# nathanaelbosch/ODEFilters.jl

Hardware: AMD Instinct MI355X
Metric: ensemble ODE-filter steps/sec (whole node) (higher is better)
Workload: dtype f64

## Files before the change

odefilters.jl_amd/csrc/ek_kernels.h:

```cpp
#pragma once
#include <hip/hip_runtime.h>
#include "dispatch.h"
#include "smooth_rows.h"
#include "smooth_lane.h"
#include "dense_lane.h"
#include "sample_lane.h"
#include "rows_kernels.h"
#include "dense_rows.h"
#include "sample_rows.h"
#include "launch.h"
#include "wave_map.h"

namespace odef {

constexpr int kWave = 64;
inline unsigned lane_grid(long N) { return (unsigned)((N + kWave - 1) / kWave); }

__device__ __attribute__((always_inline)) inline void stagger_start(const FilterParams& P) {
  if (P.stagger > 0) {
    const int n = (int)(blockIdx.x % 16u) * P.stagger;
    for (int k = 0; k < n; ++k) __builtin_amdgcn_s_sleep(1);
  }
}
template <class RHS, int q, bool EK1, bool EVERY, bool LAG = false>
__global__ __launch_bounds__(kWave) void ek_filter_fixed_kernel(const FilterParams P) {
  const long i0 = wave_first_trajectory(blockIdx.x, gridDim.x, P.wave_map);
  stagger_start(P);
  if (i0 + threadIdx.x < P.N) filter_fixed_lane<RHS, q, EK1, EVERY, LAG>(P, i0, threadIdx.x);
}
template <class RHS, int q, bool EK1>
__global__ __launch_bounds__(kWave) void ek_filter_adaptive_kernel(const FilterParams P) {
  const long i0 = (long)blockIdx.x * kWave;
  if (i0 + threadIdx.x < P.N) filter_adaptive_lane<RHS, q, EK1>(P, i0, threadIdx.x);
}
template <class RHS, int q, bool EVERY, bool LAG>
__global__ __launch_bounds__(kWave) void ek_filter_fixed_mv_kernel(const FilterParams P) {
  const long i0 = wave_first_trajectory(blockIdx.x, gridDim.x, P.wave_map);
  stagger_start(P);
  if (i0 + threadIdx.x < P.N) filter_fixed_lane<RHS, q, false, EVERY, LAG, true>(P, i0, threadIdx.x);
}
template <class RHS, int q>
__global__ __launch_bounds__(kWave) void ek_filter_adaptive_mv_kernel(const FilterParams P) {
  const long i0 = (long)blockIdx.x * kWave;
  if (i0 + threadIdx.x < P.N) filter_adaptive_lane<RHS, q, false, true>(P, i0, threadIdx.x);
}
template <class RHS, int q, bool LAG>
__global__ __launch_bounds__(kWave) void ek_filter_fixed_ieks_kernel(const FilterParams P) {
  const long i0 = wave_first_trajectory(blockIdx.x, gridDim.x, P.wave_map);
  stagger_start(P);
  if (i0 + threadIdx.x < P.N) filter_fixed_lane<RHS, q, true, true, LAG, false, true>(P, i0, threadIdx.x);
}

template <int D>
struct SmoothTeam {
  static constexpr int lanes = (D <= 16) ? 16 : 32;
  static unsigned grid(long items) { return (unsigned)((items + kWave / lanes - 1) / (kWave / lanes)); }
};
template <int d, int q, bool MV>
__device__ __attribute__((always_inline)) inline void smooth_team_entry(const SmoothParams& P) {
  constexpr int D = d * (q + 1), TEAM = SmoothTeam<D>::lanes, TPB = kWave / TEAM;
  using W = RowsWs<d, q + 1>;
  __shared__ double lds[TPB * W::size];
  const int team = threadIdx.x / TEAM, tid = threadIdx.x % TEAM;
  const long i = (long)blockIdx.x * TPB + team;
  RowState<D> st;
  if (i < P.N) smooth_rows_lane<d, q, TEAM, MV>(P, i, tid, lds + team * W::size, &st);
}
template <int d, int q>
__global__ __launch_bounds__(kWave) __attribute__((amdgpu_num_vgpr(128))) void rts_smooth_kernel(const SmoothParams P) {
  smooth_team_entry<d, q, false>(P);
}
template <int d, int q>
__global__ __launch_bounds__(kWave) __attribute__((amdgpu_num_vgpr(128))) void rts_smooth_mv_kernel(const SmoothParams P) {
  smooth_team_entry<d, q, true>(P);
}
constexpr int kSmoothLaneMaxD = 12;
constexpr long kSmoothLaneMinN = 6144;
inline long smooth_lane_min_n() { return env_long("ODEF_SMOOTH_LANE_MIN_N", kSmoothLaneMinN); }
constexpr long kFilterLagMaxN = kFilterRowsMaxN;
inline long filter_lag_max_n() { return env_long("ODEF_FILTER_LAG_MAX_N", kFilterLagMaxN); }
static_assert(kWaveMapLanes == kWave, "wave_map.h counts trajectories in wavefronts of the lane kernels");
constexpr long kWaveMapDefault = 1;
inline int wave_map_mode() { return (int)env_long("ODEF_WAVE_MAP", kWaveMapDefault); }
template <int d, int q, bool ADAPT>
__global__ __launch_bounds__(kWave) void rts_smooth_lane_kernel(const SmoothParams P) {
  constexpr int D = d * (q + 1), TRI = D * (D + 1) / 2;
  __shared__ double lds[TRI * kWave];
  const long i0 = (long)blockIdx.x * kWave;
  const LaneMem xl{lds + threadIdx.x, kWave};
  const bool valid = i0 + threadIdx.x < P.N;
  long n_hi = P.n_save;
  if constexpr (ADAPT) n_hi = wave_uniform_max(valid ? (long)P.nsaved[i0 + threadIdx.x] : 0, valid);
  if (valid) smooth_lane_v2<d, q, ADAPT>(P, i0, threadIdx.x, xl, n_hi);
}

template <int d, int q>
__global__ __launch_bounds__(kWave) void dense_output_kernel(const DenseParams P) {
  constexpr int D = d * (q + 1), TRI = D * (D + 1) / 2;
  __shared__ double lds[TRI * kWave];
  const long i = (long)blockIdx.x * kWave + threadIdx.x;
  const LaneMem xl{lds + threadIdx.x, kWave};
  if (i < P.N) dense_lane<d, q>(P, i, (long)blockIdx.y, xl);
}
template <int d, int q>
__global__ __launch_bounds__(kWave) void dense_output_mv_kernel(const DenseParams P) {
  constexpr int D = d * (q + 1), TRI = D * (D + 1) / 2;
  __shared__ double lds[TRI * kWave];
  const long i = (long)blockIdx.x * kWave + threadIdx.x;
  const LaneMem xl{lds + threadIdx.x, kWave};
  if (i < P.N) dense_lane<d, q, true>(P, i, (long)blockIdx.y, xl);
}
template <int d, int q, bool MV>
__device__ __attribute__((always_inline)) inline void dense_team_entry(const DenseParams& P) {
  constexpr int D = d * (q + 1), TEAM = SmoothTeam<D>::lanes, TPB = kWave / TEAM;
  using W = RowsWs<d, q + 1>;
  __shared__ double lds[TPB * W::size];
  const int team = threadIdx.x / TEAM, tid = threadIdx.x % TEAM;
  const long it = (long)blockIdx.x * TPB + team;
  RowState<D> st;
  if (it < P.N * P.n_q) dense_rows_lane<d, q, TEAM, MV>(P, it % P.N, it / P.N, tid, lds + team * W::size, &st);
}
template <int d, int q>
__global__ __launch_bounds__(kWave) __attribute__((amdgpu_num_vgpr(128))) void dense_rows_kernel(const DenseParams P) {
  dense_team_entry<d, q, false>(P);
}
template <int d, int q>
__global__ __launch_bounds__(kWave) __attribute__((amdgpu_num_vgpr(128))) void dense_rows_mv_kernel(const DenseParams P) {
  dense_team_entry<d, q, true>(P);
}

template <int d, int q>
__global__ __launch_bounds__(kWave) void sample_kernel(const SampleParams P) {
  constexpr int D = d * (q + 1), TRI = D * (D + 1) / 2;
  __shared__ double lds[TRI * kWave];
  const long i = (long)blockIdx.x * kWave + threadIdx.x;
  const LaneMem xl{lds + threadIdx.x, kWave};
  const bool valid = i < P.N;
  const long n_hi = (P.adaptive && !P.tq) ? wave_uniform_max(valid ? (long)P.nsaved[i] : 0, valid) : P.n_save;
  if (valid) sample_lane<d, q>(P, i, (long)blockIdx.y, xl, n_hi);
}
template <int d, int q>
__global__ __launch_bounds__(kWave) void sample_mv_kernel(const SampleParams P) {
  constexpr int D = d * (q + 1), TRI = D * (D + 1) / 2;
  __shared__ double lds[TRI * kWave];
  const long i = (long)blockIdx.x * kWave + threadIdx.x;
  const LaneMem xl{lds + threadIdx.x, kWave};
  const bool valid = i < P.N;
  const long n_hi = (P.adaptive && !P.tq) ? wave_uniform_max(valid ? (long)P.nsaved[i] : 0, valid) : P.n_save;
  if (valid) sample_lane<d, q, true>(P, i, (long)blockIdx.y, xl, n_hi);
}
template <int d, int q, bool MV>
__device__ __attribute__((always_inline)) inline void sample_team_entry(const SampleParams& P) {
  constexpr int D = d * (q + 1), TEAM = SmoothTeam<D>::lanes, TPB = kWave / TEAM;
  using W = RowsWs<d, q + 1>;
  __shared__ double lds[TPB * W::size];
  const int team = threadIdx.x / TEAM, tid = threadIdx.x % TEAM;
  const long it = (long)blockIdx.x * TPB + team;
  RowState<D> st;
  if (it < P.N * P.n_samples) sample_rows_lane<d, q, TEAM, MV>(P, it % P.N, it / P.N, tid, lds + team * W::size, &st);
}
template <int d, int q>
__global__ __launch_bounds__(kWave) __attribute__((amdgpu_num_vgpr(128))) void sample_rows_kernel(const SampleParams P) {
  sample_team_entry<d, q, false>(P);
}
template <int d, int q>
__global__ __launch_bounds__(kWave) __attribute__((amdgpu_num_vgpr(128))) void sample_rows_mv_kernel(const SampleParams P) {
  sample_team_entry<d, q, true>(P);
}

template <bool WITH_MV = true>
struct LaunchDenseT {
  const DenseParams& P;
  hipStream_t s;
  int rc = 0;
  template <int d, int q>
  void operator()() {
    if (P.mv) {
      if constexpr (WITH_MV) launch<d, q, true>();
      else rc = -2;
      return;
    }
    launch<d, q, false>();
  }
  template <int d, int q, bool MV>
  void launch() {
    constexpr int D = d * (q + 1);
    if constexpr (D <= kSmoothLaneMaxD) {
      const dim3 grid(lane_grid(P.N), (unsigned)P.n_q);
      if constexpr (MV) hipLaunchKernelGGL((dense_output_mv_kernel<d, q>), grid, dim3(kWave), 0, s, P);
      else hipLaunchKernelGGL((dense_output_kernel<d, q>), grid, dim3(kWave), 0, s, P);
    } else if constexpr (D <= 32) {
      const dim3 grid(SmoothTeam<D>::grid(P.N * P.n_q));
      if constexpr (MV) hipLaunchKernelGGL((dense_rows_mv_kernel<d, q>), grid, dim3(kWave), 0, s, P);
      else hipLaunchKernelGGL((dense_rows_kernel<d, q>), grid, dim3(kWave), 0, s, P);
    } else {
      rc = MV ? -2 : -3;
    }
  }
};
template <bool WITH_MV = true>
struct LaunchSampleT {
  const SampleParams& P;
  hipStream_t s;
  int rc = 0;
  template <int d, int q>
  void operator()() {
    if (P.mv) {
      if constexpr (WITH_MV) launch<d, q, true>();
      else rc = -2;
      return;
    }
    launch<d, q, false>();
  }
  template <int d, int q, bool MV>
  void launch() {
    constexpr int D = d * (q + 1);
    if constexpr (D <= kSmoothLaneMaxD) {
      const dim3 grid(lane_grid(P.N), (unsigned)P.n_samples);
      if constexpr (MV) hipLaunchKernelGGL((sample_mv_kernel<d, q>), grid, dim3(kWave), 0, s, P);
      else hipLaunchKernelGGL((sample_kernel<d, q>), grid, dim3(kWave), 0, s, P);
    } else if constexpr (D <= 32) {
      const dim3 grid(SmoothTeam<D>::grid(P.N * P.n_samples));
      if constexpr (MV) hipLaunchKernelGGL((sample_rows_mv_kernel<d, q>), grid, dim3(kWave), 0, s, P);
      else hipLaunchKernelGGL((sample_rows_kernel<d, q>), grid, dim3(kWave), 0, s, P);
    } else {
      rc = MV ? -2 : -3;
    }
  }
};
template <bool WITH_MV = true>
struct LaunchSmoothT {
  const SmoothParams& P;
  hipStream_t s;
  int rc = 0;
  template <int d, int q>
  void operator()() {
    if (P.mv) {
      if constexpr (WITH_MV && d * (q + 1) <= 32) launch<d, q, true>();
      else rc = -2;
      return;
    }
    launch<d, q, false>();
  }
  template <int d, int q, bool MV>
  void launch() {
    constexpr int D = d * (q + 1);
    if constexpr (!MV && D <= kRowsMaxD) {
      if (P.N < smooth_rows_max_n()) {
        const dim3 grid(rows_grid(P.N));
        note_kernel("odef::rts_smooth_bcast_kernel<%d, %d, %s>", d, q, tf(P.adaptive));
        if (P.adaptive) hipLaunchKernelGGL((rts_smooth_bcast_kernel<d, q, true>), grid, dim3(kRowsBlock), 0, s, P);
        else hipLaunchKernelGGL((rts_smooth_bcast_kernel<d, q, false>), grid, dim3(kRowsBlock), 0, s, P);
        return;
      }
    }
    if constexpr (!MV && D <= kSmoothLaneMaxD) {
      if (P.N >= smooth_lane_min_n()) {
        const dim3 grid(lane_grid(P.N));
        note_kernel("odef::rts_smooth_lane_kernel<%d, %d, %s>", d, q, tf(P.adaptive));
        if (P.adaptive) hipLaunchKernelGGL((rts_smooth_lane_kernel<d, q, true>), grid, dim3(kWave), 0, s, P);
        else hipLaunchKernelGGL((rts_smooth_lane_kernel<d, q, false>), grid, dim3(kWave), 0, s, P);
        return;
      }
    }
    const dim3 grid(SmoothTeam<D>::grid(P.N));
    note_kernel(MV ? "odef::rts_smooth_mv_kernel<%d, %d>" : "odef::rts_smooth_kernel<%d, %d>", d, q);
    if constexpr (MV) hipLaunchKernelGGL((rts_smooth_mv_kernel<d, q>), grid, dim3(kWave), 0, s, P);
    else hipLaunchKernelGGL((rts_smooth_kernel<d, q>), grid, dim3(kWave), 0, s, P);
  }
};
template <bool WITH_MV = true, bool WITH_IEKS = true>
struct LaunchFilterT {
  const FilterParams& P;
  int adaptive;
  hipStream_t s;
  int rc = 0;
  enum Mode { kScalar, kMv, kIeks };
  template <class RHS, int q, bool EK1>
  void operator()() {
    const bool mv = P.fixed_diffusion >= 3;
    if (P.lin) {
      if constexpr (WITH_IEKS && EK1) {
        if (!adaptive && P.everystep && !mv) return launch<RHS, q, EK1, kIeks>();
      }
      rc = -2;
    } else if (mv) {
      if constexpr (WITH_MV && !EK1) launch<RHS, q, EK1, kMv>();
      else rc = -2;
    } else {
      launch<RHS, q, EK1, kScalar>();
    }
  }
  template <class RHS, int q, bool EK1, Mode M>
  void launch() {
    if constexpr (RHS::d * (q + 1) <= kRowsMaxD && M != kMv) {
      if (P.N < filter_rows_max_n()) {
        const dim3 grid(rows_grid(P.N));
        if constexpr (M == kIeks) {
          note_kernel("odef::ek_filter_rows_ieks_kernel<odef::%s, %d>", RHS::name, q);
          hipLaunchKernelGGL((ek_filter_rows_ieks_kernel<RHS, q>), grid, dim3(kRowsBlock), 0, s, P);
        } else if (adaptive) {
          note_kernel("odef::ek_filter_rows_adaptive_kernel<odef::%s, %d, %s>", RHS::name, q, tf(EK1));
          hipLaunchKernelGGL((ek_filter_rows_adaptive_kernel<RHS, q, EK1>), grid, dim3(kRowsBlock), 0, s, P);
        } else {
          note_kernel("odef::ek_filter_rows_kernel<odef::%s, %d, %s, %s>", RHS::name, q, tf(EK1), tf(P.everystep));
          if (P.everystep) hipLaunchKernelGGL((ek_filter_rows_kernel<RHS, q, EK1, true>), grid, dim3(kRowsBlock), 0, s, P);
          else hipLaunchKernelGGL((ek_filter_rows_kernel<RHS, q, EK1, false>), grid, dim3(kRowsBlock), 0, s, P);
        }
        return;
      }
    }
    const dim3 grid(lane_grid(P.N));
    if constexpr (M != kIeks) {
      if (adaptive) {
        if constexpr (M == kMv) {
          note_kernel("odef::ek_filter_adaptive_mv_kernel<odef::%s, %d>", RHS::name, q);
          hipLaunchKernelGGL((ek_filter_adaptive_mv_kernel<RHS, q>), grid, dim3(kWave), 0, s, P);
        } else {
          note_kernel("odef::ek_filter_adaptive_kernel<odef::%s, %d, %s>", RHS::name, q, tf(EK1));
          hipLaunchKernelGGL((ek_filter_adaptive_kernel<RHS, q, EK1>), grid, dim3(kWave), 0, s, P);
        }
        return;
      }
    }
    const bool lag = P.everystep && P.N < filter_lag_max_n();
    FilterParams Pw = P;
    Pw.wave_map = wave_map_mode();
    if constexpr (M == kIeks) {
      note_kernel("odef::ek_filter_fixed_ieks_kernel<odef::%s, %d, %s>", RHS::name, q, tf(lag));
      if (lag) hipLaunchKernelGGL((ek_filter_fixed_ieks_kernel<RHS, q, true>), grid, dim3(kWave), 0, s, Pw);
      else hipLaunchKernelGGL((ek_filter_fixed_ieks_kernel<RHS, q, false>), grid, dim3(kWave), 0, s, Pw);
    } else if constexpr (M == kMv) {
      note_kernel("odef::ek_filter_fixed_mv_kernel<odef::%s, %d, %s, %s>", RHS::name, q, tf(P.everystep), tf(lag));
      if (lag) hipLaunchKernelGGL((ek_filter_fixed_mv_kernel<RHS, q, true, true>), grid, dim3(kWave), 0, s, Pw);
      else if (P.everystep) hipLaunchKernelGGL((ek_filter_fixed_mv_kernel<RHS, q, true, false>), grid, dim3(kWave), 0, s, Pw);
      else hipLaunchKernelGGL((ek_filter_fixed_mv_kernel<RHS, q, false, false>), grid, dim3(kWave), 0, s, Pw);
    } else {
      note_kernel("odef::ek_filter_fixed_kernel<odef::%s, %d, %s, %s, %s>", RHS::name, q, tf(EK1), tf(P.everystep), tf(lag));
      if (lag) hipLaunchKernelGGL((ek_filter_fixed_kernel<RHS, q, EK1, true, true>), grid, dim3(kWave), 0, s, Pw);
      else if (P.everystep) hipLaunchKernelGGL((ek_filter_fixed_kernel<RHS, q, EK1, true>), grid, dim3(kWave), 0, s, Pw);
      else hipLaunchKernelGGL((ek_filter_fixed_kernel<RHS, q, EK1, false>), grid, dim3(kWave), 0, s, Pw);
    }
  }
};

template <class RHS, int ONLYQ = 0, bool ONLYEK1 = false, bool WITH_MV = true, bool WITH_IEKS = true>
int lane_filter(int q, int ek1, const FilterParams& P, hipStream_t s, int adaptive, double*, size_t, long*) {
  LaunchFilterT<WITH_MV, WITH_IEKS> f{P, adaptive, s};
  const int rc = dispatch_order<RHS, ONLYQ, ONLYEK1>(q, ek1, f);
  return rc ? rc : f.rc;
}
template <int d, int ONLYQ = 0, bool WITH_MV = true>
int lane_smooth(int q, const SmoothParams& P, double*, hipStream_t s) {
  LaunchSmoothT<WITH_MV> f{P, s};
  const int rc = dispatch_smooth_order<d, ONLYQ>(q, f);
  return rc ? rc : f.rc;
}
template <int d, int ONLYQ = 0, bool WITH_MV = true>
int lane_dense(int q, const DenseParams& P, double*, hipStream_t s) {
  LaunchDenseT<WITH_MV> f{P, s};
  const int rc = dispatch_smooth_order<d, ONLYQ>(q, f);
  return rc ? rc : f.rc;
}
template <int d, int ONLYQ = 0, bool WITH_MV = true>
int lane_sample(int q, const SampleParams& P, double*, hipStream_t s) {
  LaunchSampleT<WITH_MV> f{P, s};
  const int rc = dispatch_smooth_order<d, ONLYQ>(q, f);
  return rc ? rc : f.rc;
}
extern template int lane_smooth<2>(int, const SmoothParams&, double*, hipStream_t);
extern template int lane_dense<2>(int, const DenseParams&, double*, hipStream_t);
extern template int lane_sample<2>(int, const SampleParams&, double*, hipStream_t);
extern template int lane_smooth<3>(int, const SmoothParams&, double*, hipStream_t);
extern template int lane_dense<3>(int, const DenseParams&, double*, hipStream_t);
extern template int lane_sample<3>(int, const SampleParams&, double*, hipStream_t);

}
```

odefilters.jl_amd/csrc/smooth_lane.h:

```cpp
#pragma once
#include "ek_lane.h"

namespace odef {

struct LaneMem {
  double* base;
  int stride;
  __device__ inline double get(int k) const { return base[k * stride]; }
  __device__ inline void set(int k, double v) const { base[k * stride] = v; }
};

template <int D>
__device__ inline void two_sided_inverse(double (&S)[D * (D + 1) / 2], const double (&L)[D * (D + 1) / 2], const double (&dinv)[D]) {
  static_for<0, D>([&](auto kc) {
    constexpr int k = decltype(kc)::value;
    const double inv = dinv[k];
    const double tkk = S[tri(k, k)] * inv * inv;
    S[tri(k, k)] = tkk;
    const double htkk = -0.5 * tkk;
#pragma unroll
    for (int j = 0; j < k; ++j) S[tri(k, j)] *= inv;
    double b[D];
#pragma unroll
    for (int i = k + 1; i < D; ++i) {
      const double lik = L[tri(i, k)];
      b[i] = __builtin_fma(lik, htkk, S[tri(i, k)] * inv);
#pragma unroll
      for (int j = 0; j < k; ++j) S[tri(i, j)] = __builtin_fma(-lik, S[tri(k, j)], S[tri(i, j)]);
    }
#pragma unroll
    for (int i = k + 1; i < D; ++i) {
      const double lik = L[tri(i, k)];
#pragma unroll
      for (int j = k + 1; j <= i; ++j)
        S[tri(i, j)] = __builtin_fma(-L[tri(j, k)], b[i], __builtin_fma(-lik, b[j], S[tri(i, j)]));
      S[tri(i, k)] = __builtin_fma(lik, htkk, b[i]);
    }
    ODEF_SCHED_FENCE();
  });
  static_for<0, D>([&](auto kc) {
    constexpr int k = D - 1 - decltype(kc)::value;
    const double inv = dinv[k];
    double t[D];
#pragma unroll
    for (int j = 0; j < D; ++j) {
      double s = S[symidx(k, j)];
#pragma unroll
      for (int i = k + 1; i < D; ++i) s -= L[tri(i, k)] * S[symidx(i, j)];
      t[j] = s;
    }
    double tk = t[k];
#pragma unroll
    for (int i = k + 1; i < D; ++i) tk -= L[tri(i, k)] * t[i];
#pragma unroll
    for (int j = 0; j < D; ++j)
      if (j != k) S[symidx(k, j)] = t[j] * inv;
    S[tri(k, k)] = tk * inv * inv;
    ODEF_SCHED_FENCE();
  });
}

template <int d, int NB>
__device__ inline void congruence_At_inplace(const PriorConsts& pc, double (&X)[d * NB * (d * NB + 1) / 2]) {
  constexpr int D = d * NB;
#pragma unroll
  for (int J = NB - 1; J >= 1; --J) {
    double Wd[d][d];
#pragma unroll
    for (int a = 0; a < d; ++a)
#pragma unroll
      for (int b = 0; b < d; ++b) {
        double t = X[symidx(J * d + a, J * d + b)];
#pragma unroll
        for (int j = 0; j < J; ++j) t += pc.At[j][J] * X[symidx(j * d + a, J * d + b)];
        Wd[a][b] = t;
      }
#pragma unroll
    for (int a = 0; a < d; ++a)
#pragma unroll
      for (int c = 0; c < D; ++c) {
        if (c / d == J) continue;
        double t = X[symidx(J * d + a, c)];
#pragma unroll
        for (int j = 0; j < J; ++j) t += pc.At[j][J] * X[symidx(j * d + a, c)];
        X[symidx(J * d + a, c)] = t;
      }
#pragma unroll
    for (int a = 0; a < d; ++a)
#pragma unroll
      for (int b = 0; b <= a; ++b) {
        double t = Wd[a][b];
#pragma unroll
        for (int j = 0; j < J; ++j) t += pc.At[j][J] * X[symidx(J * d + a, j * d + b)];
        X[tri(J * d + a, J * d + b)] = t;
      }
  }
}

template <int d, int NB, class CovSink, class Sig = double>
__device__ inline void rts_step_core(const PriorConsts& pc, const double (&pij)[NB], const double (&mt)[d * NB],
                                     double (&B)[d * NB * (d * NB + 1) / 2], double (&Cs)[d * NB * (d * NB + 1) / 2],
                                     const double (&msn)[d * NB], Sig sigma2, const LaneMem& xl,
                                     double (&ms_out)[d * NB], CovSink& sink) {
  constexpr int D = d * NB, TRI = D * (D + 1) / 2;
  double dl[D];
#pragma unroll
  for (int J = 0; J < NB; ++J)
#pragma unroll
    for (int a = 0; a < d; ++a) {
      double t = mt[J * d + a];
#pragma unroll
      for (int j = J + 1; j < NB; ++j) t += pc.At[J][j] * mt[j * d + a];
      dl[J * d + a] = msn[J * d + a] - t;
    }
  ODEF_SCHED_FENCE();
  predict_cov_inplace<d, NB>(pc, B, sigma2);
  ODEF_SCHED_FENCE();
#pragma unroll
  for (int k = 0; k < TRI; ++k) Cs[k] -= B[k];
  int fixes = 0;
  double dinv[D];
  chol_packed<D>(B, fixes, dinv);
  ODEF_SCHED_FENCE();
#pragma unroll
  for (int k = 0; k < D; ++k) {
    double t = dl[k];
#pragma unroll
    for (int c = 0; c < k; ++c) t -= B[tri(k, c)] * dl[c];
    dl[k] = t * dinv[k];
  }
#pragma unroll
  for (int k = D - 1; k >= 0; --k) {
    double t = dl[k];
#pragma unroll
    for (int c = k + 1; c < D; ++c) t -= B[tri(c, k)] * dl[c];
    dl[k] = t * dinv[k];
  }
  double wv[D];
#pragma unroll
  for (int K = 0; K < NB; ++K)
#pragma unroll
    for (int b = 0; b < d; ++b) {
      double t = dl[K * d + b];
#pragma unroll
      for (int j = 0; j < K; ++j) t += pc.At[j][K] * dl[j * d + b];
      wv[K * d + b] = t;
    }
  ODEF_SCHED_FENCE();
  two_sided_inverse<D>(Cs, B, dinv);
  ODEF_SCHED_FENCE();
  congruence_At_inplace<d, NB>(pc, Cs);
  ODEF_SCHED_FENCE();
  static_for<0, D>([&](auto ac) {
    constexpr int a = decltype(ac)::value;
    double xa[D], u[D];
#pragma unroll
    for (int c = 0; c < D; ++c) xa[c] = xl.get(symidx(a, c));
    double mnew = mt[a];
#pragma unroll
    for (int c = 0; c < D; ++c) mnew += xa[c] * wv[c];
    ms_out[a] = mnew * pij[a / d];
#pragma unroll
    for (int c = 0; c < D; ++c) {
      double t = 0.0;
#pragma unroll
      for (int k = 0; k < D; ++k) t += xa[k] * Cs[symidx(k, c)];
      u[c] = t;
    }
#pragma unroll
    for (int b = 0; b <= a; ++b) {
      double t = xa[b];
#pragma unroll
      for (int k = 0; k < D; ++k) t += u[k] * xl.get(symidx(k, b));
      sink(tri(a, b), t * (pij[a / d] * pij[b / d]));
    }
    ODEF_SCHED_FENCE();
  });
}

__device__ inline long wave_uniform_max(long v, bool valid) {
#ifdef ODEF_HOST_EMUL
  (void)valid;
  return v;
#else
  int x = valid ? (int)v : 0;
  for (int m = 32; m >= 1; m >>= 1) {
    const int y = __shfl_xor(x, m, 64);
    x = x > y ? x : y;
  }
  return (long)__builtin_amdgcn_readfirstlane(x);
#endif
}

#ifdef ODEF_HOST_EMUL
inline double* agpr_file() {
  static thread_local double f[256];
  return f;
}
template <int R>
inline void aput(double v) { agpr_file()[R] = v; }
template <int R>
inline double aget() { return agpr_file()[R]; }
inline void agpr_file_claim() {}
#else
template <int R>
__device__ __attribute__((always_inline)) inline void aput(double v) {
  static_assert(R >= 0 && R < 128, "a lane has 256 AGPRs = 128 doubles");
  asm volatile("v_accvgpr_write_b32 a[%1], %0" ::"v"(__double2loint(v)), "n"(2 * R));
  asm volatile("v_accvgpr_write_b32 a[%1], %0" ::"v"(__double2hiint(v)), "n"(2 * R + 1));
}
template <int R>
__device__ __attribute__((always_inline)) inline double aget() {
  static_assert(R >= 0 && R < 128, "a lane has 256 AGPRs = 128 doubles");
  int lo, hi;
  asm volatile("v_accvgpr_read_b32 %0, a[%1]" : "=v"(lo) : "n"(2 * R));
  asm volatile("v_accvgpr_read_b32 %0, a[%1]" : "=v"(hi) : "n"(2 * R + 1));
  return __hiloint2double(hi, lo);
}
__device__ __attribute__((always_inline)) inline void agpr_file_claim() { asm volatile("" ::: "a255"); }
#endif

template <int n>
__device__ __attribute__((always_inline)) inline void pin(double (&a)[n]) {
#ifndef ODEF_HOST_EMUL
#pragma unroll
  for (int k = 0; k < n; ++k) asm volatile("" : "+v"(a[k]));
#else
  (void)a;
#endif
}

template <int D>
__device__ inline void ldl_packed_lane(double (&B)[D * (D + 1) / 2], double (&dinv)[D]) {
  static_for<0, D>([&](auto kc) {
    constexpr int k = decltype(kc)::value;
    const double piv = B[tri(k, k)];
    const bool ok = piv > 0.0;
    const double inv = ok ? rcp_pos(ok ? piv : 1.0) : 0.0;
    dinv[k] = inv;
    double v[D];
#pragma unroll
    for (int i = k + 1; i < D; ++i) {
      v[i] = B[tri(i, k)];
      B[tri(i, k)] = v[i] * inv;
    }
#pragma unroll
    for (int j = k + 1; j < D; ++j)
#pragma unroll
      for (int i = j; i < D; ++i) B[tri(i, j)] = __builtin_fma(-B[tri(i, k)], v[j], B[tri(i, j)]);
  });
}

template <int D, int LS>
__device__ inline void two_sided_inverse_parked(double (&S)[D * (D + 1) / 2]) {
  static_for<0, D>([&](auto kc) {
    constexpr int k = decltype(kc)::value;
    double lc[D];
    static_for<k + 1, D>([&](auto ic) { lc[decltype(ic)::value] = aget<LS + tri(decltype(ic)::value, k)>(); });
    const double htkk = -0.5 * S[tri(k, k)];
    double b[D];
#pragma unroll
    for (int i = k + 1; i < D; ++i) {
      b[i] = __builtin_fma(lc[i], htkk, S[tri(i, k)]);
#pragma unroll
      for (int j = 0; j < k; ++j) S[tri(i, j)] = __builtin_fma(-lc[i], S[tri(k, j)], S[tri(i, j)]);
    }
#pragma unroll
    for (int i = k + 1; i < D; ++i) {
#pragma unroll
      for (int j = k + 1; j <= i; ++j) S[tri(i, j)] = __builtin_fma(-lc[j], b[i], __builtin_fma(-lc[i], b[j], S[tri(i, j)]));
      S[tri(i, k)] = __builtin_fma(lc[i], htkk, b[i]);
    }
    pin(S);
    ODEF_SCHED_FENCE();
  });
  {
    double di[D];
    static_for<0, D>([&](auto kc) { di[decltype(kc)::value] = aget<LS + tri(decltype(kc)::value, decltype(kc)::value)>(); });
#pragma unroll
    for (int i = 0; i < D; ++i) {
#pragma unroll
      for (int j = 0; j < i; ++j) S[tri(i, j)] = (S[tri(i, j)] * di[i]) * di[j];
      S[tri(i, i)] = __builtin_fma(S[tri(i, i)] * di[i], di[i], -di[i]);
    }
    pin(S);
    ODEF_SCHED_FENCE();
  }
  static_for<0, D>([&](auto kc) {
    constexpr int k = D - 1 - decltype(kc)::value;
    double lc[D];
    static_for<k + 1, D>([&](auto ic) { lc[decltype(ic)::value] = aget<LS + tri(decltype(ic)::value, k)>(); });
    double t[D];
#pragma unroll
    for (int j = 0; j < D; ++j) {
      double s = S[symidx(k, j)];
#pragma unroll
      for (int i = k + 1; i < D; ++i) s -= lc[i] * S[symidx(i, j)];
      t[j] = s;
    }
    double tk = t[k];
#pragma unroll
    for (int i = k + 1; i < D; ++i) tk -= lc[i] * t[i];
#pragma unroll
    for (int j = 0; j < D; ++j)
      if (j != k) S[symidx(k, j)] = t[j];
    S[tri(k, k)] = tk;
    pin(S);
    ODEF_SCHED_FENCE();
  });
}

template <int d, int q, bool ADAPT>
__device__ inline void smooth_lane_v2(const SmoothParams& P, long i0, unsigned lane, const LaneMem& xl, long n_hi) {
  constexpr int NB = q + 1, D = d * NB, TRI = D * (D + 1) / 2;
  constexpr int MS = 128 - (TRI + D), VS = MS + TRI;
  static_assert(MS >= 0, "the AGPR file holds 128 doubles");
  agpr_file_claim();
  const long i = i0 + lane;
  const long n = ADAPT ? (long)P.nsaved[i] : P.n_save;
  const size_t N = (size_t)P.N;
  const PriorConsts& pc = P.pc;
  for (int w = 0; w < 2; ++w) {
    const long s = w == 0 ? 0 : n - 1;
    double c[TRI], m[D];
    const double* src = P.cov + ((size_t)s * TRI) * N + i;
#pragma unroll
    for (int k = 0; k < TRI; ++k) c[k] = src[(size_t)k * N];
#pragma unroll
    for (int k = 0; k < D; ++k) m[k] = P.mean[((size_t)s * D + k) * N + i];
    ODEF_SCHED_FENCE();
    double* dst = P.scov + ((size_t)s * TRI) * N + i;
#pragma unroll
    for (int k = 0; k < TRI; ++k) dst[(size_t)k * N] = c[k];
#pragma unroll
    for (int k = 0; k < D; ++k) P.smean[((size_t)s * D + k) * N + i] = m[k];
    static_for<0, TRI>([&](auto kc) { aput<MS + decltype(kc)::value>(c[decltype(kc)::value]); });
    static_for<0, D>([&](auto kc) { aput<VS + decltype(kc)::value>(m[decltype(kc)::value]); });
  }
  bool nan_seen = false;
  for (long s = n_hi - 2; s >= 1; --s) {
    if constexpr (ADAPT) {
      if (s > n - 2) continue;
    }
    double h, pj[NB], pij[NB];
    if constexpr (ADAPT) {
      h = P.tsave[(size_t)(s + 1) * N + i] - P.tsave[(size_t)s * N + i];
      double val = (h != 0.0) ? precond_val<q>(h) : 1.0;
#pragma unroll
      for (int J = 0; J < NB; ++J) {
        pj[J] = val;
        pij[J] = 1.0 / val;
        val *= h;
      }
    } else {
      h = uniform_load(P.hs + s);
      const GlobalTab tab{P.ptab + (size_t)uniform_load(P.tab_idx + s) * kTabStride};
#pragma unroll
      for (int J = 0; J < NB; ++J) {
        pj[J] = tab[kTabPJ + J];
        pij[J] = tab[kTabPIJ + J];
      }
    }
    RowStore sm(P.smean + ((size_t)s * D) * N + i0, N, D, lane), sc(P.scov + ((size_t)s * TRI) * N + i0, N, TRI, lane);
    if (h == 0.0) {
      static_for<0, D>([&](auto kc) { sm.put(aget<VS + decltype(kc)::value>()); });
      static_for<0, TRI>([&](auto kc) { sc.put(aget<MS + decltype(kc)::value>()); });
      continue;
    }
    const double sigma2 = P.diff[(size_t)(s + 1) * N + i];
    double mt[D], B[TRI];
    {
      RowLoad lc(P.cov + ((size_t)s * TRI) * N + i0, N, TRI, lane), lm(P.mean + ((size_t)s * D) * N + i0, N, D, lane);
#pragma unroll
      for (int k = 0; k < TRI; ++k) B[k] = lc.get();
#pragma unroll
      for (int k = 0; k < D; ++k) mt[k] = lm.get();
    }
    ODEF_SCHED_FENCE();
#pragma unroll
    for (int k = 0; k < D; ++k) mt[k] *= pj[k / d];
#pragma unroll
    for (int a = 0; a < D; ++a)
#pragma unroll
      for (int b = 0; b <= a; ++b) {
        const double x = B[tri(a, b)] * (pj[a / d] * pj[b / d]);
        xl.set(tri(a, b), x);
        B[tri(a, b)] = x;
      }
    pin(B);
    double dl[D];
    static_for<0, D>([&](auto kc) { dl[decltype(kc)::value] = aget<VS + decltype(kc)::value>(); });
#pragma unroll
    for (int J = 0; J < NB; ++J)
#pragma unroll
      for (int a = 0; a < d; ++a) {
        double t = mt[J * d + a];
#pragma unroll
        for (int j = J + 1; j < NB; ++j) t += pc.At[J][j] * mt[j * d + a];
        dl[J * d + a] = pj[J] * dl[J * d + a] - t;
      }
    pin(dl);
    ODEF_SCHED_FENCE();
    predict_cov_inplace<d, NB>(pc, B, sigma2);
    pin(B);
    ODEF_SCHED_FENCE();
    double dinv[D];
    ldl_packed_lane<D>(B, dinv);
    pin(B);
    pin(dinv);
    ODEF_SCHED_FENCE();
#pragma unroll
    for (int k = 0; k < D; ++k) {
      double t = dl[k];
#pragma unroll
      for (int c = 0; c < k; ++c) t -= B[tri(k, c)] * dl[c];
      dl[k] = t;
    }
#pragma unroll
    for (int k = 0; k < D; ++k) dl[k] *= dinv[k];
#pragma unroll
    for (int k = D - 1; k >= 0; --k) {
      double t = dl[k];
#pragma unroll
      for (int c = k + 1; c < D; ++c) t -= B[tri(c, k)] * dl[c];
      dl[k] = t;
    }
#pragma unroll
    for (int K = NB - 1; K >= 1; --K)
#pragma unroll
      for (int b = 0; b < d; ++b)
#pragma unroll
        for (int j = 0; j < K; ++j) dl[K * d + b] += pc.At[j][K] * dl[j * d + b];
#pragma unroll
    for (int a = 0; a < D; ++a)
#pragma unroll
      for (int c = 0; c <= a; ++c) {
        const double x = xl.get(tri(a, c));
        mt[a] += x * dl[c];
        if (c != a) mt[c] += x * dl[a];
      }
    static_for<0, D>([&](auto kc) {
      constexpr int k = decltype(kc)::value;
      const double v = mt[k] * pij[k / d];
      nan_seen = nan_seen || !(v == v);
      sm.put(v);
      aput<VS + k>(v);
    });
    ODEF_SCHED_FENCE();
    double S[TRI];
    static_for<0, TRI>([&](auto kc) {
      constexpr int k = decltype(kc)::value;
      constexpr int a = [] { int r = 0; while ((r + 1) * (r + 2) / 2 <= k) ++r; return r; }();
      constexpr int b = k - a * (a + 1) / 2;
      S[k] = aget<MS + k>();
      aput<MS + k>(a == b ? dinv[a] : B[k]);
      S[k] *= pj[a / d] * pj[b / d];
    });
    pin(S);
    ODEF_SCHED_FENCE();
    two_sided_inverse_parked<D, MS>(S);
    pin(S);
    ODEF_SCHED_FENCE();
    congruence_At_inplace<d, NB>(pc, S);
    pin(S);
    ODEF_SCHED_FENCE();
    auto rows = [&](auto a0c, auto nrc) {
      constexpr int a0 = decltype(a0c)::value, nr = decltype(nrc)::value;
      double u[nr][D];
#pragma unroll
      for (int r = 0; r < nr; ++r) {
        double xa[D];
#pragma unroll
        for (int c = 0; c < D; ++c) xa[c] = xl.get(symidx(a0 + r, c));
#pragma unroll
        for (int c = 0; c < D; ++c) {
          double t = 0.0;
#pragma unroll
          for (int k = 0; k < D; ++k) t += xa[k] * S[symidx(k, c)];
          u[r][c] = t;
        }
      }
      RowStore st[2] = {sc.at_row(tri(a0, 0)), sc.at_row(tri(a0 + nr - 1, 0))};
      static_for<0, a0 + nr>([&](auto bc) {
        constexpr int b = decltype(bc)::value;
        double col[D];
#pragma unroll
        for (int k = 0; k < D; ++k) col[k] = xl.get(symidx(k, b));
        static_for<0, nr>([&](auto rc) {
          constexpr int a = a0 + decltype(rc)::value;
          if constexpr (b <= a) {
            double t = col[a];
#pragma unroll
            for (int k = 0; k < D; ++k) t += u[a - a0][k] * col[k];
            const double v = t * (pij[a / d] * pij[b / d]);
            st[a - a0].put(v);
            aput<MS + tri(a, b)>(v);
          }
        });
      });
      ODEF_SCHED_FENCE();
    };
    static_for<0, D / 2>([&](auto pc_) { rows(std::integral_constant<int, 2 * decltype(pc_)::value>{}, std::integral_constant<int, 2>{}); });
    if constexpr (D % 2 == 1) rows(std::integral_constant<int, D - 1>{}, std::integral_constant<int, 1>{});
  }
  if (nan_seen) P.retcode[i] = 3;
}

}
```

Before: 8.464 billion.

## Swap smoother LDS roles: keep X in registers, stream S through LDS ring

In the lane RTS smoother's final X + X·S·X update, the packed covariance X is copied into registers and S is written into the per-lane LDS slot. The X·S product is then built by streaming S pairs through a small prefetch ring, so each S element feeds both symmetric contributions, and the second product reads X from registers instead of re-reading LDS columns. The aim is fewer LDS reads and better overlap of LDS latency with FMAs, at the cost of more register pressure from holding X[TRI]. The old path stays selectable through an env var, and optional cycle-stamp instrumentation is added under a macro.

Result: no change. 8.459 billion (-0.1%).

```diff
diff --git a/odefilters.jl_amd/csrc/ek_kernels.h b/odefilters.jl_amd/csrc/ek_kernels.h
--- a/odefilters.jl_amd/csrc/ek_kernels.h
+++ b/odefilters.jl_amd/csrc/ek_kernels.h
@@ -82,7 +82,8 @@
 static_assert(kWaveMapLanes == kWave, "wave_map.h counts trajectories in wavefronts of the lane kernels");
 constexpr long kWaveMapDefault = 1;
 inline int wave_map_mode() { return (int)env_long("ODEF_WAVE_MAP", kWaveMapDefault); }
-template <int d, int q, bool ADAPT>
+inline bool smooth_xwx_mode() { return env_long("ODEF_SMOOTH_XWX", kSmoothXwxDefault ? 1 : 0) != 0; }
+template <int d, int q, bool ADAPT, bool XWX = kSmoothXwxDefault>
 __global__ __launch_bounds__(kWave) void rts_smooth_lane_kernel(const SmoothParams P) {
   constexpr int D = d * (q + 1), TRI = D * (D + 1) / 2;
   __shared__ double lds[TRI * kWave];
@@ -91,7 +92,7 @@
   const bool valid = i0 + threadIdx.x < P.N;
   long n_hi = P.n_save;
   if constexpr (ADAPT) n_hi = wave_uniform_max(valid ? (long)P.nsaved[i0 + threadIdx.x] : 0, valid);
-  if (valid) smooth_lane_v2<d, q, ADAPT>(P, i0, threadIdx.x, xl, n_hi);
+  if (valid) smooth_lane_v2<d, q, ADAPT, XWX>(P, i0, threadIdx.x, xl, n_hi);
 }
 
 template <int d, int q>
@@ -228,7 +229,7 @@
     }
   }
 };
-template <bool WITH_MV = true>
+template <bool WITH_MV = true, bool BOTH_XWX = true>
 struct LaunchSmoothT {
   const SmoothParams& P;
   hipStream_t s;
@@ -258,6 +259,13 @@
       if (P.N >= smooth_lane_min_n()) {
         const dim3 grid(lane_grid(P.N));
         note_kernel("odef::rts_smooth_lane_kernel<%d, %d, %s>", d, q, tf(P.adaptive));
+        if constexpr (BOTH_XWX) {
+          if (smooth_xwx_mode() != kSmoothXwxDefault) {
+            if (P.adaptive) hipLaunchKernelGGL((rts_smooth_lane_kernel<d, q, true, !kSmoothXwxDefault>), grid, dim3(kWave), 0, s, P);
+            else hipLaunchKernelGGL((rts_smooth_lane_kernel<d, q, false, !kSmoothXwxDefault>), grid, dim3(kWave), 0, s, P);
+            return;
+          }
+        }
         if (P.adaptive) hipLaunchKernelGGL((rts_smooth_lane_kernel<d, q, true>), grid, dim3(kWave), 0, s, P);
         else hipLaunchKernelGGL((rts_smooth_lane_kernel<d, q, false>), grid, dim3(kWave), 0, s, P);
         return;
@@ -352,7 +360,7 @@
 }
 template <int d, int ONLYQ = 0, bool WITH_MV = true>
 int lane_smooth(int q, const SmoothParams& P, double*, hipStream_t s) {
-  LaunchSmoothT<WITH_MV> f{P, s};
+  LaunchSmoothT<WITH_MV, ONLYQ == 0> f{P, s};
   const int rc = dispatch_smooth_order<d, ONLYQ>(q, f);
   return rc ? rc : f.rc;
 }
diff --git a/odefilters.jl_amd/csrc/smooth_lane.h b/odefilters.jl_amd/csrc/smooth_lane.h
--- a/odefilters.jl_amd/csrc/smooth_lane.h
+++ b/odefilters.jl_amd/csrc/smooth_lane.h
@@ -310,9 +310,39 @@
   });
 }
 
-template <int d, int q, bool ADAPT>
+constexpr int tri_row(int k) {
+  int r = 0;
+  while ((r + 1) * (r + 2) / 2 <= k) ++r;
+  return r;
+}
+
+constexpr bool kSmoothXwxDefault = true;
+constexpr int kLdsAhead = 4;
+
+#ifdef ODEF_SMOOTH_LANE_STAMPS
+__device__ unsigned long long g_lane_stamps[16];
+#define ODEF_LSTAMP(k)                                              \
+  do {                                                              \
+    ODEF_SCHED_FENCE();                                             \
+    const unsigned long long now_ = __builtin_readcyclecounter();   \
+    if ((k) >= 0) st_acc[(k) < 0 ? 0 : (k)] += now_ - st_t0;        \
+    st_t0 = now_;                                                   \
+    ODEF_SCHED_FENCE();                                             \
+  } while (0)
+#else
+#define ODEF_LSTAMP(k)
+#endif
+
+template <int d, int q, bool ADAPT, bool XWX = kSmoothXwxDefault>
 __device__ inline void smooth_lane_v2(const SmoothParams& P, long i0, unsigned lane, const LaneMem& xl, long n_hi) {
   constexpr int NB = q + 1, D = d * NB, TRI = D * (D + 1) / 2;
+  constexpr int NP = (TRI + 1) / 2, AHEAD = kLdsAhead < NP ? kLdsAhead : NP;
+  double ring[AHEAD][2];
+  auto fetch = [&](auto slotc, auto pc_) {
+    constexpr int slot = decltype(slotc)::value, p = decltype(pc_)::value;
+    ring[slot][0] = xl.get(2 * p);
+    if constexpr (2 * p + 1 < TRI) ring[slot][1] = xl.get(2 * p + 1);
+  };
   constexpr int MS = 128 - (TRI + D), VS = MS + TRI;
   static_assert(MS >= 0, "the AGPR file holds 128 doubles");
   agpr_file_claim();
@@ -338,7 +368,11 @@
     static_for<0, D>([&](auto kc) { aput<VS + decltype(kc)::value>(m[decltype(kc)::value]); });
   }
   bool nan_seen = false;
+#ifdef ODEF_SMOOTH_LANE_STAMPS
+  unsigned long long st_acc[8] = {0, 0, 0, 0, 0, 0, 0, 0}, st_t0 = 0;
+#endif
   for (long s = n_hi - 2; s >= 1; --s) {
+    ODEF_LSTAMP(-1);
     if constexpr (ADAPT) {
       if (s > n - 2) continue;
     }
@@ -377,6 +411,11 @@
       for (int k = 0; k < D; ++k) mt[k] = lm.get();
     }
     ODEF_SCHED_FENCE();
+#ifdef ODEF_SMOOTH_LANE_STAMPS
+    pin(B);
+    pin(mt);
+#endif
+    ODEF_LSTAMP(0);
 #pragma unroll
     for (int k = 0; k < D; ++k) mt[k] *= pj[k / d];
 #pragma unroll
@@ -388,6 +427,7 @@
         B[tri(a, b)] = x;
       }
     pin(B);
+    ODEF_LSTAMP(1);
     double dl[D];
     static_for<0, D>([&](auto kc) { dl[decltype(kc)::value] = aget<VS + decltype(kc)::value>(); });
 #pragma unroll
@@ -409,6 +449,7 @@
     pin(B);
     pin(dinv);
     ODEF_SCHED_FENCE();
+    ODEF_LSTAMP(2);
 #pragma unroll
     for (int k = 0; k < D; ++k) {
       double t = dl[k];
@@ -447,11 +488,11 @@
       aput<VS + k>(v);
     });
     ODEF_SCHED_FENCE();
+    ODEF_LSTAMP(3);
     double S[TRI];
     static_for<0, TRI>([&](auto kc) {
       constexpr int k = decltype(kc)::value;
-      constexpr int a = [] { int r = 0; while ((r + 1) * (r + 2) / 2 <= k) ++r; return r; }();
-      constexpr int b = k - a * (a + 1) / 2;
+      constexpr int a = tri_row(k), b = k - tri(a, 0);
       S[k] = aget<MS + k>();
       aput<MS + k>(a == b ? dinv[a] : B[k]);
       S[k] *= pj[a / d] * pj[b / d];
@@ -461,48 +502,130 @@
     two_sided_inverse_parked<D, MS>(S);
     pin(S);
     ODEF_SCHED_FENCE();
+    ODEF_LSTAMP(4);
     congruence_At_inplace<d, NB>(pc, S);
     pin(S);
     ODEF_SCHED_FENCE();
-    auto rows = [&](auto a0c, auto nrc) {
-      constexpr int a0 = decltype(a0c)::value, nr = decltype(nrc)::value;
-      double u[nr][D];
-#pragma unroll
-      for (int r = 0; r < nr; ++r) {
-        double xa[D];
-#pragma unroll
-        for (int c = 0; c < D; ++c) xa[c] = xl.get(symidx(a0 + r, c));
-#pragma unroll
-        for (int c = 0; c < D; ++c) {
-          double t = 0.0;
-#pragma unroll
-          for (int k = 0; k < D; ++k) t += xa[k] * S[symidx(k, c)];
-          u[r][c] = t;
-        }
-      }
-      RowStore st[2] = {sc.at_row(tri(a0, 0)), sc.at_row(tri(a0 + nr - 1, 0))};
-      static_for<0, a0 + nr>([&](auto bc) {
-        constexpr int b = decltype(bc)::value;
-        double col[D];
-#pragma unroll
-        for (int k = 0; k < D; ++k) col[k] = xl.get(symidx(k, b));
-        static_for<0, nr>([&](auto rc) {
-          constexpr int a = a0 + decltype(rc)::value;
-          if constexpr (b <= a) {
-            double t = col[a];
-#pragma unroll
-            for (int k = 0; k < D; ++k) t += u[a - a0][k] * col[k];
-            const double v = t * (pij[a / d] * pij[b / d]);
-            st[a - a0].put(v);
-            aput<MS + tri(a, b)>(v);
-          }
+    ODEF_LSTAMP(5);
+    if constexpr (XWX) {
+      double X[TRI];
+      static_for<0, NP>([&](auto pc_) {
+        constexpr int p = decltype(pc_)::value;
+        static_for<0, 2>([&](auto ec) {
+          constexpr int k = 2 * p + decltype(ec)::value;
+          if constexpr (k < TRI) X[k] = xl.get(k);
         });
+        static_for<0, 2>([&](auto ec) {
+          constexpr int k = 2 * p + decltype(ec)::value;
+          if constexpr (k < TRI) xl.set(k, S[k]);
+        });
+        if constexpr (p % 4 == 3) ODEF_SCHED_FENCE();
       });
       ODEF_SCHED_FENCE();
-    };
-    static_for<0, D / 2>([&](auto pc_) { rows(std::integral_constant<int, 2 * decltype(pc_)::value>{}, std::integral_constant<int, 2>{}); });
-    if constexpr (D % 2 == 1) rows(std::integral_constant<int, D - 1>{}, std::integral_constant<int, 1>{});
+      static_for<0, AHEAD>([&](auto pc_) {
+        constexpr int p = decltype(pc_)::value;
+        ring[p][0] = S[2 * p];
+        if constexpr (2 * p + 1 < TRI) ring[p][1] = S[2 * p + 1];
+      });
+      ODEF_SCHED_FENCE();
+      auto rows = [&](auto a0c, auto nrc, auto passc, auto lastc) {
+        constexpr int a0 = decltype(a0c)::value, nr = decltype(nrc)::value;
+        constexpr int g0 = decltype(passc)::value * NP;
+        constexpr bool last = decltype(lastc)::value;
+        double u[nr][D];
+#pragma unroll
+        for (int r = 0; r < nr; ++r)
+#pragma unroll
+          for (int c = 0; c < D; ++c) u[r][c] = 0.0;
+        static_for<0, NP>([&](auto pc_) {
+          constexpr int p = decltype(pc_)::value, slot = (g0 + p) % AHEAD;
+          static_for<0, 2>([&](auto ec) {
+            constexpr int k = 2 * p + decltype(ec)::value;
+            if constexpr (k < TRI) {
+              constexpr int i = tri_row(k), j = k - tri(i, 0);
+              const double w = ring[slot][k - 2 * p];
+#pragma unroll
+              for (int r = 0; r < nr; ++r) u[r][j] += X[symidx(a0 + r, i)] * w;
+              if constexpr (i != j) {
+#pragma unroll
+                for (int r = 0; r < nr; ++r) u[r][i] += X[symidx(a0 + r, j)] * w;
+              }
+            }
+          });
+          if constexpr (p + AHEAD < NP) fetch(std::integral_constant<int, slot>{}, std::integral_constant<int, p + AHEAD>{});
+          else if constexpr (!last) fetch(std::integral_constant<int, slot>{}, std::integral_constant<int, p + AHEAD - NP>{});
+          ODEF_SCHED_FENCE();
+        });
+        RowStore st[2] = {sc.at_row(tri(a0, 0)), sc.at_row(tri(a0 + nr - 1, 0))};
+        static_for<0, a0 + nr>([&](auto bc) {
+          constexpr int b = decltype(bc)::value;
+          static_for<0, nr>([&](auto rc) {
+            constexpr int a = a0 + decltype(rc)::value;
+            if constexpr (b <= a) {
+              double t = X[symidx(a, b)];
+#pragma unroll
+              for (int k = 0; k < D; ++k) t += u[a - a0][k] * X[symidx(k, b)];
+              const double v = t * (pij[a / d] * pij[b / d]);
+              st[a - a0].put(v);
+              aput<MS + tri(a, b)>(v);
+            }
+          });
+        });
+        ODEF_SCHED_FENCE();
+      };
+      constexpr int NPASS = (D + 1) / 2;
+      static_for<0, D / 2>([&](auto pc_) {
+        constexpr int p = decltype(pc_)::value;
+        rows(std::integral_constant<int, 2 * p>{}, std::integral_constant<int, 2>{}, pc_, std::bool_constant<p == NPASS - 1>{});
+      });
+      if constexpr (D % 2 == 1)
+        rows(std::integral_constant<int, D - 1>{}, std::integral_constant<int, 1>{}, std::integral_constant<int, NPASS - 1>{}, std::true_type{});
+    } else {
+      auto rows = [&](auto a0c, auto nrc) {
+        constexpr int a0 = decltype(a0c)::value, nr = decltype(nrc)::value;
+        double u[nr][D];
+#pragma unroll
+        for (int r = 0; r < nr; ++r) {
+          double xa[D];
+#pragma unroll
+          for (int c = 0; c < D; ++c) xa[c] = xl.get(symidx(a0 + r, c));
+#pragma unroll
+          for (int c = 0; c < D; ++c) {
+            double t = 0.0;
+#pragma unroll
+            for (int k = 0; k < D; ++k) t += xa[k] * S[symidx(k, c)];
+            u[r][c] = t;
+          }
+        }
+        RowStore st[2] = {sc.at_row(tri(a0, 0)), sc.at_row(tri(a0 + nr - 1, 0))};
+        static_for<0, a0 + nr>([&](auto bc) {
+          constexpr int b = decltype(bc)::value;
+          double col[D];
+#pragma unroll
+          for (int k = 0; k < D; ++k) col[k] = xl.get(symidx(k, b));
+          static_for<0, nr>([&](auto rc) {
+            constexpr int a = a0 + decltype(rc)::value;
+            if constexpr (b <= a) {
+              double t = col[a];
+#pragma unroll
+              for (int k = 0; k < D; ++k) t += u[a - a0][k] * col[k];
+              const double v = t * (pij[a / d] * pij[b / d]);
+              st[a - a0].put(v);
+              aput<MS + tri(a, b)>(v);
+            }
+          });
+        });
+        ODEF_SCHED_FENCE();
+      };
+      static_for<0, D / 2>([&](auto pc_) { rows(std::integral_constant<int, 2 * decltype(pc_)::value>{}, std::integral_constant<int, 2>{}); });
+      if constexpr (D % 2 == 1) rows(std::integral_constant<int, D - 1>{}, std::integral_constant<int, 1>{});
+    }
+    ODEF_LSTAMP(6);
   }
+#ifdef ODEF_SMOOTH_LANE_STAMPS
+  if (i == 0)
+    for (int k = 0; k < 8; ++k) g_lane_stamps[k] = st_acc[k];
+#endif
   if (nan_seen) P.retcode[i] = 3;
 }
 
```
